# PaddlePaddle/Anakin

Hardware: AMD Instinct MI355X
Metric: ResNet50 INT8 images/sec + p50 latency @ batch 1/8, 1×MI355X (higher is better)
Workload: dtype int8

## Files before the change

### anakin_amd/build.py

```python
import os
import subprocess
import sys

HERE = os.path.dirname(os.path.abspath(__file__))
CSRC = os.path.join(HERE, "csrc")
LIB = os.path.join(HERE, "libsaber_mi355x.so")
SOURCES = ["conv_igemm.hip", "elementwise.hip", "fc_small.hip", "conv1x1_chain.hip", "conv_chain_coop.hip", "conv_stage_coop.hip", "stage_xcd.hip", "conv3x3_b3h.hip", "conv1x1_pw.hip", "conv1x1_pwk.hip", "conv_stem_f32.hip", "fc_f32_splitk.hip", "conv_dw3x3.hip", "conv_group3x3.hip", "conv_sep.hip"] + \
    ["api_%s.hip" % n for n in ("conv", "select", "autotune", "ops", "chain", "sep", "stage", "net", "net_optimize", "net_autotune", "capture", "gemm", "streams")] + \
    ["igemm_m%d_e%d.hip" % me for me in [(0, 0), (0, 1), (0, 2), (0, 3), (0, 4), (1, 0), (1, 1), (1, 2), (1, 3), (2, 3), (3, 3)]] + \
    ["igemm_dma_m%d_e%d.hip" % me for me in [(0, 0), (0, 1), (0, 2), (0, 3), (0, 4), (2, 3)]] + \
    ["halo_e%d.hip" % e for e in range(4)] + ["img_e%d.hip" % e for e in (0, 1, 3)] + ["stem_e%d.hip" % e for e in range(4)] + ["stem_pool.hip"]
FLAGS = ["--offload-arch=gfx950", "-O3", "-std=c++17", "-fPIC", "-ffp-contract=off", "-fno-fast-math",
         "-Wno-unused-result", "-mllvm", "-amdgpu-mfma-vgpr-form"]


def _stale(obj, deps):
    if not os.path.exists(obj):
        return True
    t = os.path.getmtime(obj)
    return any(os.path.getmtime(d) > t for d in deps)


def build(force=False, verbose=False):
    hipcc = os.environ.get("HIPCC", "/opt/rocm/bin/hipcc")
    objdir = os.path.join(HERE, "build")
    os.makedirs(objdir, exist_ok=True)
    import glob
    headers = sorted(glob.glob(os.path.join(CSRC, "*.h"))) + [os.path.join(HERE, "..", "include", "saber_hip.h")]
    objs = []
    procs = []
    for src in SOURCES:
        sp = os.path.join(CSRC, src)
        obj = os.path.join(objdir, src.replace(".hip", ".o"))
        objs.append(obj)
        deps = [h for h in headers if src.startswith("api_") or os.path.basename(h) != "api_internal.h"]
        if force or _stale(obj, [sp] + deps):
            cmd = [hipcc] + FLAGS + ["-c", sp, "-o", obj]
            if verbose:
                print(" ".join(cmd))
            procs.append((src, subprocess.Popen(cmd)))
    for src, p in procs:
        if p.wait() != 0:
            raise RuntimeError("hipcc failed on " + src)
    if force or procs or _stale(LIB, objs):
        cmd = [hipcc, "--offload-arch=gfx950", "-shared", "-o", LIB] + objs
        if verbose:
            print(" ".join(cmd))
        subprocess.check_call(cmd)
    return LIB


def build_cpp_tests(verbose=False):
    import glob
    root = os.path.dirname(HERE)
    build()
    subprocess.check_call(["make", "-s", "-C", os.path.join(root, "oracle"), "oracle"])
    hipcc = os.environ.get("HIPCC", "/opt/rocm/bin/hipcc")
    outs = []
    for src in sorted(glob.glob(os.path.join(root, "tests", "cpp", "*.cpp"))):
        out = src[:-4] + ".bin"
        deps = [src, os.path.join(root, "include", "saber_mi355x.hpp"), os.path.join(root, "include", "saber_mi355x_impl.h"), os.path.join(root, "include", "saber_hip.h"), LIB]
        if _stale(out, deps):
            cmd = [hipcc, "--offload-arch=gfx950", "-O2", "-std=c++17", "-I" + os.path.join(root, "include"), src, "-o", out,
                   "-L" + HERE, "-lsaber_mi355x", "-L" + os.path.join(root, "oracle"), "-lsaber_oracle",
                   "-Wl,-rpath,$ORIGIN/../../anakin_amd", "-Wl,-rpath,$ORIGIN/../../oracle", "-Wno-unused-result", "-mllvm", "-amdgpu-mfma-vgpr-form"]
            if verbose:
                print(" ".join(cmd))
            subprocess.check_call(cmd)
        outs.append(out)
    return outs


if __name__ == "__main__":
    print(build(force="--force" in sys.argv, verbose=True))
```

### anakin_amd/csrc/api_stage.hip

```cpp
#include "api_internal.h"

struct saber_hip_stage {
    std::vector<saber_hip_conv*> convs;
    std::vector<StagePhase> phases;
    DevBuf<uint8_t> d_phases, d_w, d_prm;
    DevBuf<unsigned long long> d_sync, d_trace;
    int n_barriers = 0, n_tensors = 0, n_img = 0, h = 0, w = 0;
    size_t lds_bytes = 0;
};

namespace {
constexpr int kSyncWords = 16 * 17 + 16;

bool stage_conv_ok(const saber_hip_conv* o) {
    const saber_hip_conv_desc& d = o->d;
    const bool k1 = d.kh == 1 && d.kw == 1 && d.pad_h == 0 && d.pad_w == 0;
    const bool k3 = d.kh == 3 && d.kw == 3 && d.pad_h == 1 && d.pad_w == 1;
    const bool res_ok = d.res_mode == SABER_HIP_RES_NONE ||
                        (d.res_mode == SABER_HIP_RES_ELTWISE && d.out_dtype == SABER_HIP_S8 &&
                         (!d.res_has_dtype || d.res_dtype == SABER_HIP_S8) && d.res_stride <= 1);
    return o->is_i8 && o->weights_set && o->algo == ALGO_IGEMM_I8 && o->epi == EPI_I8_CONV && (k1 || k3) && d.stride_h == 1 &&
           d.stride_w == 1 && d.dil_h == 1 && d.dil_w == 1 && d.group == 1 && !o->pair_k2 && !o->pool_fused && !o->pool2 &&
           !o->pre_quant && !o->pre_pad && o->c_eff == d.c && d.act_negative_slope == 0.f && d.in_layout == SABER_HIP_NHWC &&
           d.out_layout == SABER_HIP_NHWC && (d.out_dtype == SABER_HIP_S8 || d.out_dtype == SABER_HIP_U8) && res_ok &&
// ... 53 lines not shown
        if (i == 0) { st->n_img = d.n; st->h = d.h; st->w = d.w; }
        if (d.n != st->n_img || d.h != st->h || d.w != st->w || d.h * d.w > 64) return fail(SABER_HIP_INVALID_VALUE, "stage: all phases run on the same n x h x w, h * w <= 64");
        const int slots[4] = {ph[i].in, ph[i].out, elt ? ph[i].res : 0, ph[i].pool >= 0 ? ph[i].pool : 0};
        for (int s : slots)
            if (s < 0 || s >= STAGE_MAX_TENSORS) return fail(SABER_HIP_INVALID_VALUE, "stage: tensor slot out of range");
        if (ph[i].out == ph[i].in || (elt && ph[i].out == ph[i].res) || written[ph[i].out])
            return fail(SABER_HIP_INVALID_VALUE, "stage: every phase writes a slot of its own (no in-place, no rewrite)");
        const int taps = d.kh * d.kw, ksteps = d.c * taps / 64;
        const int nt = (d.k / 16 + 31) / 32;
        StagePhase p;
        std::memset(&p, 0, sizeof p);
        if (ksteps % 4 || !stage_xcd_type(nt, ksteps / 4, taps == 9, &p.type))
            return fail(SABER_HIP_INVALID_VALUE, "stage: no kernel variant for " + std::to_string(d.c) + " -> " + std::to_string(d.k) + (taps == 9 ? " 3x3" : " 1x1"));
        p.cin = d.c; p.cout = d.k;
        p.in_t = ph[i].in; p.out_t = ph[i].out; p.res_t = elt ? ph[i].res : -1;
        p.in_u8 = o->x_dtype == DT_U8;
        p.relu = d.act == SABER_HIP_ACT_RELU;
        p.out_u8 = d.out_dtype == SABER_HIP_U8;
        p.elt = elt;
        p.res_relu = d.res_act == SABER_HIP_ACT_RELU;
        p.coeff_conv = d.coeff_conv; p.scale_conv = o->out_scale; p.coeff_res = d.coeff_res; p.scale_res = d.scale_res;
        p.barrier = dirty[p.in_t] || (elt && dirty[p.res_t]);
        if (p.barrier) {
            std::fill(dirty.begin(), dirty.end(), 0);
            st->n_barriers += 1;
        }
        p.reload = (p.barrier || p.in_t != prev_in || i == 0) ? 1 : 0;
        prev_in = p.in_t;
        dirty[p.out_t] = written[p.out_t] = 1;
        p.pch = (unsigned)(d.c / 16 + 1);
        p.mg_pch = (unsigned)((0x100000000ull + p.pch - 1) / p.pch);
        const size_t a64 = ((size_t)(d.h * d.w + 1) * p.pch + 63) / 64 * 64;
        p.red_chunk = (int)a64;
        lds_chunks = std::max(lds_chunks, a64 + (size_t)4 * nt * 4 * 64 + (size_t)4 * nt * 4);
        p.pool_t = ph[i].pool;
        p.pool_idiv = 1.0f / (float)(d.h * d.w);
        p.w_chunk = (unsigned)(wbytes.size() / 16);
        pack_stage_weights(o, nt, ksteps / 4, wbytes);
        p.prm_chunk = (unsigned)(pbytes.size() / 16);
        const int kpad = 32 * nt * 16;
        const size_t base = pbytes.size();
        pbytes.resize(base + (size_t)kpad / 4 * 48, 0);
        for (int k = 0; k < d.k; ++k) {
            uint8_t* q = pbytes.data() + base + (size_t)(k / 4) * 48;
            ((float*)q)[k % 4] = o->scale_host.empty() ? 1.f : o->scale_host[k];
            ((float*)q)[4 + k % 4] = (o->has_bias && !o->bias_p_host.empty()) ? o->bias_p_host[k] : 0.f;
            ((int*)q)[8 + k % 4] = o->comp_host.empty() ? 0 : o->comp_host[k];
        }
        st->n_tensors = std::max(st->n_tensors, std::max(std::max(p.in_t, p.pool_t), std::max(p.out_t, p.res_t)) + 1);
        st->phases.push_back(p);
        st->convs.push_back(o);
    }
    st->lds_bytes = xcd_resident ? std::max<size_t>(lds_chunks * 16, 81 * 1024) : lds_chunks * 16;
    if (st->lds_bytes > 160 * 1024 - 64) return fail(SABER_HIP_UNIMPL, "stage: the image does not fit in LDS");
    std::vector<uint8_t> pt((const uint8_t*)st->phases.data(), (const uint8_t*)st->phases.data() + st->phases.size() * sizeof(StagePhase));
    hipError_t e = st->d_phases.upload(pt);
    if (e == hipSuccess) e = st->d_w.upload(wbytes);
    if (e == hipSuccess) e = st->d_prm.upload(pbytes);
    if (e == hipSuccess && xcd_resident) e = st->d_sync.alloc_zero(kSyncWords);
    if (e != hipSuccess) return hip_fail(e, "stage: device copies");
    if (!zero_page()) return fail(SABER_HIP_RUNTIME_ERROR, "stage: zero page");
    *out = st.release();
    return SABER_HIP_OK;
}
}

bool img_conv_ok(const saber_hip_conv* op) {
    if (!stage_conv_ok(op) || op->d.h * op->d.w > 64) return false;
    const int taps = op->d.kh * op->d.kw, ksteps = op->d.c * taps / 64;
    int type = 0;
    return ksteps % 4 == 0 && stage_xcd_type((op->d.k / 16 + 31) / 32, ksteps / 4, taps == 9, &type);
}
int img_conv_prepare(saber_hip_conv* op) {
    if (op->img_stage) return SABER_HIP_OK;
    if (!img_conv_ok(op)) return fail(SABER_HIP_INVALID_VALUE, "image-resident kernel: 1x1 / 3x3 stride-1 INT8 conv on <= 64 pixels per image with ResNet res5 channel shapes");
    const StageSpec sp = {op, 0, 1, op->d.res_mode == SABER_HIP_RES_ELTWISE ? 2 : -1, op->gpool ? 3 : -1};
    return stage_build(&sp, 1, false, &op->img_stage);
}
int img_conv_run(saber_hip_conv* op, const void* x, void* y, const void* res, void* y_pool, hipStream_t stream) {
    saber_hip_stage* st = op->img_stage;
    if (!st) return fail(SABER_HIP_INVALID_VALUE, "image-resident kernel selected without its buffers (set_tile / autotune build them)");
    const StagePhase& p = st->phases[0];
    if (!x || !y || (p.elt && !res) || (p.pool_t >= 0 && !y_pool)) return fail(SABER_HIP_INVALID_VALUE, "null tensor");
    StageKArgs k;
    std::memset(&k, 0, sizeof k);
    k.phases = (const StagePhase*)st->d_phases.p;
    k.weights = st->d_w.p; k.prm = st->d_prm.p; k.zero = zero_page();
    k.n_phases = 1;
    k.n_img = st->n_img; k.H = st->h; k.W = st->w;
    k.t[0] = const_cast<void*>(x); k.t[1] = y; k.t[2] = const_cast<void*>(res); k.t[3] = y_pool;
    HIP_TRY(launch_img_conv(k, st->lds_bytes, stream));
    return SABER_HIP_OK;
}
void img_conv_release(saber_hip_conv* op) {
    delete op->img_stage;
    op->img_stage = nullptr;
}

int saber_hip_stage_num_tensors(const saber_hip_stage_t* st) { return st ? st->n_tensors : 0; }

int saber_hip_stage_run(saber_hip_stage_t* st, void* const* tensors, int n_tensors, saber_hip_stream_t stream) {
    if (g_capture) return capture_unsupported("saber_hip_stage_run");
    if (!st || !tensors || n_tensors < st->n_tensors) return fail(SABER_HIP_INVALID_VALUE, "stage: tensor table too short");
    StageKArgs k;
    std::memset(&k, 0, sizeof k);
    k.phases = (const StagePhase*)st->d_phases.p;
    k.weights = st->d_w.p; k.prm = st->d_prm.p; k.zero = zero_page();
    k.sync = st->d_sync.p;
    k.n_phases = (int)st->phases.size(); k.n_barriers = st->n_barriers;
    k.n_img = st->n_img; k.H = st->h; k.W = st->w;
    k.trace = st->d_trace.p;
    for (int i = 0; i < st->n_tensors; ++i) k.t[i] = tensors[i];
    for (const StagePhase& p : st->phases)
        if (!k.t[p.in_t] || !k.t[p.out_t] || (p.elt && !k.t[p.res_t])) return fail(SABER_HIP_INVALID_VALUE, "stage: null tensor");
    HIP_TRY(launch_stage_xcd(k, st->lds_bytes, (hipStream_t)stream));
    return SABER_HIP_OK;
}

int saber_hip_stage_status(saber_hip_stage_t* st) {
    if (!st) return fail(SABER_HIP_INVALID_VALUE, "null argument");
    HIP_TRY(hipDeviceSynchronize());
    unsigned long long flag = 0;
    HIP_TRY(hipMemcpy(&flag, st->d_sync.p + 16 * 16, sizeof flag, hipMemcpyDeviceToHost));
    if (!flag) return SABER_HIP_OK;
    HIP_TRY(hipMemset(st->d_sync.p, 0, kSyncWords * sizeof(unsigned long long)));
    HIP_TRY(hipDeviceSynchronize());
    return fail(SABER_HIP_RUNTIME_ERROR, "stage: a workgroup gave up waiting for its XCD (the launch did not have the CUs to itself)");
}

int saber_hip_stage_trace(saber_hip_stage_t* st, unsigned long long* out, size_t cap) {
    if (!st) return fail(SABER_HIP_INVALID_VALUE, "null argument");
    const size_t n = (size_t)256 * st->phases.size() * 8;
    if (!out) {
        HIP_TRY(st->d_trace.alloc_zero(n));
        return (int)n;
    }
    if (!st->d_trace.p || cap < n) return fail(SABER_HIP_INVALID_VALUE, "stage trace: not armed / buffer too short");
    HIP_TRY(hipDeviceSynchronize());
    HIP_TRY(hipMemcpy(out, st->d_trace.p, n * sizeof(unsigned long long), hipMemcpyDeviceToHost));
    return (int)n;
}

void saber_hip_stage_destroy(saber_hip_stage_t* st) { delete st; }
```

### anakin_amd/csrc/fc_small.hip

```cpp
#include "conv_igemm_impl.h"

namespace saber_mi355x {

struct FcSoftmaxTail {
    float* prob;
    unsigned* ctr;
};
template <int KSW, bool SM, bool FENCED = false>
__device__ __forceinline__ void fc_i8_small_body(const ConvKArgs& a, const FcSoftmaxTail& t) {
    __shared__ v4i red[3][64];
    __shared__ unsigned last_flag;
    SABER_TL_DECL;
    SABER_TL(0);
    const int tid = threadIdx.x, lane = tid & 63;
    const int wave = __builtin_amdgcn_readfirstlane(tid >> 6);
    const int frow = lane & 15, fq = lane >> 4;
    const int n0 = blockIdx.x * 16;
    const int m = frow < a.M ? frow : a.M - 1;
    const char* wp = (const char*)a.w + (size_t)(n0 + frow) * a.Kg_pad + (size_t)wave * (KSW * 64) + fq * 16;
    const char* xp = (const char*)a.x + (size_t)m * a.C + (size_t)wave * (KSW * 64) + fq * 16;
    v4i wf[KSW], xf[KSW];
#pragma unroll
    for (int s = 0; s < KSW; ++s) wf[s] = *(const v4i*)(wp + s * 64);
#pragma unroll
    for (int s = 0; s < KSW; ++s) {
        const bool in = (wave * KSW + s) * 64 + fq * 16 < a.C;
        xf[s] = *(const v4i*)(in ? xp + s * 64 : (const char*)a.zero);
    }
    const int kb = n0 + fq * 4;
    ChanParams<4> cp;
    load_chan_params<4>(a, kb, cp);
    const int xmask = a.in_u8 ? (int)0x80808080u : 0;
    SABER_TL(1);
    v4i acc = {0, 0, 0, 0};
#pragma unroll
    for (int s = 0; s < KSW; ++s) {
        v4i b = xf[s];
        b.x ^= xmask; b.y ^= xmask; b.z ^= xmask; b.w ^= xmask;
        acc = mma_step(wf[s], b, acc);
    }
    SABER_TL(2);
    if (wave > 0) red[wave - 1][lane] = acc;
    __syncthreads();
    SABER_TL(3);
    if (wave == 0) {
        acc += red[0][lane];
        acc += red[1][lane];
        acc += red[2][lane];
        if (frow < a.M && kb < a.K) {
            float out[4];
#pragma unroll
            for (int r = 0; r < 4; ++r) {
                const int v = acc[r] + cp.comp[r];
                const float d = (float)v;
                if (a.epi == EPI_I8_FC_S8) out[r] = __fadd_rn(__fmul_rn(d, cp.scale[r]), cp.bias[r]);
                else out[r] = (cp.scale[r] == 1.f) ? d : __fmul_rn(cp.scale[r], d);
            }
            float* y = (float*)a.y + (size_t)frow * a.K + kb;
            if constexpr (SM) {
                for (int r = 0; r < 4; ++r)
                    if (kb + r < a.K) __hip_atomic_store(y + r, out[r], __ATOMIC_RELAXED, __HIP_MEMORY_SCOPE_AGENT);
            } else if (kb + 4 <= a.K && (a.K & 3) == 0) {
                *(float4*)y = make_float4(out[0], out[1], out[2], out[3]);
            } else {
                for (int r = 0; r < 4; ++r)
                    if (kb + r < a.K) y[r] = out[r];
            }
        }
    }
    SABER_TL(4);
    if constexpr (!SM) {
        SABER_TL_FLUSH();
        return;
    } else {
        if constexpr (FENCED) {
            asm volatile("s_waitcnt vmcnt(0)" ::: "memory");
            __syncthreads();
            if (tid == 0) {
                __builtin_amdgcn_fence(__ATOMIC_RELEASE, "agent");
                asm volatile("s_waitcnt vmcnt(0)" ::: "memory");
                last_flag = __hip_atomic_fetch_add(t.ctr, 1u, __ATOMIC_RELAXED, __HIP_MEMORY_SCOPE_AGENT) == gridDim.x - 1 ? 1u : 0u;
                if (last_flag) __builtin_amdgcn_fence(__ATOMIC_ACQUIRE, "agent");
            }
        } else if (wave == 0) {
            asm volatile("s_waitcnt vmcnt(0)" ::: "memory");
            if (lane == 0) last_flag = __hip_atomic_fetch_add(t.ctr, 1u, __ATOMIC_RELAXED, __HIP_MEMORY_SCOPE_AGENT) == gridDim.x - 1 ? 1u : 0u;
        }
        __syncthreads();
        if (!last_flag) {
            SABER_TL_FLUSH();
            return;
        }
        SABER_TL(5);
        if (tid == 0) __hip_atomic_store(t.ctr, 0u, __ATOMIC_RELAXED, __HIP_MEMORY_SCOPE_AGENT);
        constexpr int PER = 16;
        for (int row0 = wave; row0 < a.M; row0 += 8) {
            const int row1 = row0 + 4;
            const bool has1 = row1 < a.M;
            const float* y0 = (const float*)a.y + (size_t)row0 * a.K;
            const float* y1 = (const float*)a.y + (size_t)(has1 ? row1 : row0) * a.K;
            float v0[PER], v1[PER];
#pragma unroll
            for (int i = 0; i < PER; ++i) {
                const int c = lane + 64 * i;
                const int cc = c < a.K ? c : a.K - 1;
                v0[i] = __hip_atomic_load(y0 + cc, __ATOMIC_RELAXED, __HIP_MEMORY_SCOPE_SYSTEM);
                v1[i] = __hip_atomic_load(y1 + cc, __ATOMIC_RELAXED, __HIP_MEMORY_SCOPE_SYSTEM);
            }
            auto normalise = [&](float (&v)[PER], int row) {
                float mx = -3.4e38f;
#pragma unroll
                for (int i = 0; i < PER; ++i) mx = lane + 64 * i < a.K ? fmaxf(mx, v[i]) : mx;
#pragma unroll
                for (int o = 32; o > 0; o >>= 1) mx = fmaxf(mx, __shfl_xor(mx, o, 64));
                float sum = 0.f;
#pragma unroll
                for (int i = 0; i < PER; ++i) {
                    v[i] = lane + 64 * i < a.K ? expf(v[i] - mx) : 0.f;
                    sum += v[i];
                }
#pragma unroll
                for (int o = 32; o > 0; o >>= 1) sum += __shfl_xor(sum, o, 64);
                float* pr = t.prob + (size_t)row * a.K;
#pragma unroll
                for (int i = 0; i < PER; ++i)
                    if (lane + 64 * i < a.K) pr[lane + 64 * i] = v[i] / sum;
            };
            normalise(v0, row0);
            if (has1) normalise(v1, row1);
        }
        SABER_TL(6);
        SABER_TL_FLUSH();
    }
}
template <int KSW>
__global__ __launch_bounds__(256) void fc_i8_small_kernel(const ConvKArgs a) {
    fc_i8_small_body<KSW, false>(a, FcSoftmaxTail{nullptr, nullptr});
}
template <int KSW, bool FENCED>
__global__ __launch_bounds__(256) void fc_i8_small_softmax_kernel(const ConvKArgs a, const FcSoftmaxTail t) {
    fc_i8_small_body<KSW, true, FENCED>(a, t);
}

struct FcStreamArgs {
    const float* w;
    const float* x;
    float* y;
    const float* bias;
    const void* zero;
    int m, n, c, w_pitch;
    int w_rows;
    int relu;
    float neg_slope, alpha, beta;
};

template <int NS, int NW, bool PACKED>
__global__ __launch_bounds__(NW * 64) void fc_f32_stream_kernel(const FcStreamArgs a) {
    __shared__ v4f redf[NW - 1][64];
    const int tid = threadIdx.x, lane = tid & 63;
    const int wave = __builtin_amdgcn_readfirstlane(tid >> 6);
    const int frow = lane & 15, fq = lane >> 4;
    const int n0 = blockIdx.x * 16;
    const int m = frow < a.m ? frow : a.m - 1;
    const int wr = n0 + frow < a.w_rows ? n0 + frow : a.w_rows - 1;
    const int ksw = (a.c + NW * 16 - 1) / (NW * 16);
    const int k0 = wave * ksw * 16 + fq * 4;
    const float* const wrow = PACKED ? a.w + ((size_t)blockIdx.x * a.w_pitch * 64 + lane) * 4 : a.w + (size_t)wr * a.w_pitch;
    const float* const xrow = a.x + (size_t)m * a.c;
    const float* const zero = (const float*)a.zero;
    v4f acc[4];
#pragma unroll
    for (int i = 0; i < 4; ++i) acc[i] = v4f{0.f, 0.f, 0.f, 0.f};
    v4i wf[2][NS], xf[2][NS];
    auto request = [&](int b, int s0) {
#pragma unroll
        for (int s = 0; s < NS; ++s) {
            const int k = k0 + (s0 + s) * 16;
            const bool in = s0 + s < ksw && k < a.c;
            const float* wp = PACKED ? wrow + (size_t)(s0 + s < ksw ? wave * ksw + s0 + s : wave * ksw) * 256 : (in ? wrow + k : wrow);
            const float* xp = in ? xrow + k : zero;
            wf[b][s] = __builtin_nontemporal_load((const v4i*)wp);
            xf[b][s] = *(const v4i*)xp;
        }
    };
    auto multiply = [&](int b) {
#pragma unroll
        for (int s = 0; s < NS; ++s) {
            const v4f wv = __builtin_bit_cast(v4f, wf[b][s]);
            const v4f xv = __builtin_bit_cast(v4f, xf[b][s]);
            acc[0] = __builtin_amdgcn_mfma_f32_16x16x4f32(wv.x, xv.x, acc[0], 0, 0, 0);
            acc[1] = __builtin_amdgcn_mfma_f32_16x16x4f32(wv.y, xv.y, acc[1], 0, 0, 0);
            acc[2] = __builtin_amdgcn_mfma_f32_16x16x4f32(wv.z, xv.z, acc[2], 0, 0, 0);
            acc[3] = __builtin_amdgcn_mfma_f32_16x16x4f32(wv.w, xv.w, acc[3], 0, 0, 0);
        }
    };
    const int nch = (ksw + NS - 1) / NS;
    const int rot = (int)((blockIdx.x * 7u + wave * 3u) % (unsigned)nch);
    auto chunk_s0 = [&](int ci) { return ci < nch ? ((ci + rot) % nch) * NS : ksw; };
    request(0, chunk_s0(0));
    __builtin_amdgcn_sched_barrier(0);
    for (int ci = 0; ci < nch; ci += 2) {
        request(1, chunk_s0(ci + 1));
        __builtin_amdgcn_sched_barrier(0);
        multiply(0);
        __builtin_amdgcn_sched_barrier(0);
        request(0, chunk_s0(ci + 2));
        __builtin_amdgcn_sched_barrier(0);
        multiply(1);
        __builtin_amdgcn_sched_barrier(0);
    }
    v4f sum = (acc[0] + acc[1]) + (acc[2] + acc[3]);
    if (wave > 0) redf[wave - 1][lane] = sum;
    __syncthreads();
    if (wave > 0) return;
#pragma unroll
    for (int w = 0; w < NW - 1; ++w) sum += redf[w][lane];
    const int kb = n0 + fq * 4;
    if (frow >= a.m || kb >= a.n) return;
    float* y = a.y + (size_t)frow * a.n + kb;
    float out[4];
#pragma unroll
    for (int r = 0; r < 4; ++r) {
        float d = a.alpha == 1.f ? sum[r] : __fmul_rn(a.alpha, sum[r]);
// ... 87 lines not shown
#pragma unroll
    for (int r = 0; r < 4; ++r) {
        float d = a.alpha == 1.f ? sum[r] : __fmul_rn(a.alpha, sum[r]);
        if (a.bias && kb + r < a.n) d = __fadd_rn(d, a.bias[kb + r]);
        if (a.relu) d = d > 0.f ? d : (a.neg_slope == 0.f ? 0.f : __fmul_rn(d, a.neg_slope));
        if (a.beta != 0.f && kb + r < a.n) d = __fadd_rn(d, __fmul_rn(a.beta, y[r]));
        out[r] = d;
    }
    if (kb + 4 <= a.n && (a.n & 3) == 0) {
        *(float4*)y = make_float4(out[0], out[1], out[2], out[3]);
    } else {
        for (int r = 0; r < 4; ++r)
            if (kb + r < a.n) y[r] = out[r];
    }
}

bool fc_f32_small_ok(int m, int c, int kg_pad) { return m >= 1 && m <= 16 && c % 4 == 0 && c <= 65536 && kg_pad >= (c + 63) / 64 * 64; }
static hipError_t launch_fc_f32_stream(const FcStreamArgs& f, bool packed, hipStream_t s) {
    const dim3 grid((f.n + 15) / 16);
    const bool deep = (f.c + 63) / 64 >= 48;
    if (packed) {
        if (deep) hipLaunchKernelGGL((fc_f32_stream_kernel<12, 4, true>), grid, dim3(256), 0, s, f);
        else hipLaunchKernelGGL((fc_f32_stream_kernel<4, 4, true>), grid, dim3(256), 0, s, f);
    } else {
        if (deep) hipLaunchKernelGGL((fc_f32_stream_kernel<12, 4, false>), grid, dim3(256), 0, s, f);
        else hipLaunchKernelGGL((fc_f32_stream_kernel<4, 4, false>), grid, dim3(256), 0, s, f);
    }
    return hipGetLastError();
}
hipError_t launch_fc_f32_small(const ConvKArgs& a, bool packed, hipStream_t s) {
    if (!fc_f32_small_ok(a.M, a.C, a.Kg_pad)) return hipErrorInvalidValue;
    FcStreamArgs f;
    f.w = (const float*)a.w; f.x = (const float*)a.x; f.y = (float*)a.y; f.bias = a.bias; f.zero = a.zero;
    f.m = a.M; f.n = a.K; f.c = a.C;
    f.w_pitch = packed ? fc_f32_packed_steps(a.C) : a.Kg_pad;
    f.w_rows = (a.K + 15) / 16 * 16;
    f.relu = a.relu; f.neg_slope = a.neg_slope; f.alpha = 1.f; f.beta = 0.f;
    if (!packed && a.C >= 2048) {
        const dim3 grid((f.n + 15) / 16), block(256);
        if (f.m <= 8) hipLaunchKernelGGL((gemm_f32_rows_lds_kernel<8>), grid, block, 0, s, f);
        else hipLaunchKernelGGL((gemm_f32_rows_lds_kernel<16>), grid, block, 0, s, f);
        return hipGetLastError();
    }
    return launch_fc_f32_stream(f, packed, s);
}
int fc_f32_packed_steps(int c) { return 4 * ((c + 63) / 64); }
bool gemm_f32_rows_ok(int m, int k) { return m >= 1 && m <= 16 && k % 4 == 0 && k <= (1 << 24); }
hipError_t launch_gemm_f32_rows(int m, int n, int k, float alpha, const float* A, const float* B, float beta, float* C, const void* zero,
                                hipStream_t s) {
    if (!gemm_f32_rows_ok(m, k)) return hipErrorInvalidValue;
    FcStreamArgs f;
    f.w = B; f.x = A; f.y = C; f.bias = nullptr; f.zero = zero;
    f.m = m; f.n = n; f.c = k; f.w_pitch = k; f.w_rows = n;
    f.relu = 0; f.neg_slope = 0.f; f.alpha = alpha; f.beta = beta;
    static const bool gather = [] { const char* e = std::getenv("SABER_HIP_GEMM_ROWS_GATHER"); return e && e[0] == '1'; }();
    if (k >= 2048 && !gather) {
        const dim3 grid((n + 15) / 16), block(256);
        if (m <= 8) hipLaunchKernelGGL((gemm_f32_rows_lds_kernel<8>), grid, block, 0, s, f);
        else hipLaunchKernelGGL((gemm_f32_rows_lds_kernel<16>), grid, block, 0, s, f);
        return hipGetLastError();
    }
    return launch_fc_f32_stream(f, false, s);
}

bool fc_i8_small_ok(int m, int c, int kg_pad) { return m >= 1 && m <= 16 && c % 16 == 0 && c <= 4 * 16 * 64 && kg_pad >= ((c + 255) / 256) * 256; }

hipError_t launch_fc_i8_small(const ConvKArgs& a, hipStream_t s) {
    if (!fc_i8_small_ok(a.M, a.C, a.Kg_pad)) return hipErrorInvalidValue;
    const int ksw = (a.C + 255) / 256;
    dim3 grid((a.K + 15) / 16), block(256);
#define SABER_FC_CASE(n) case n: hipLaunchKernelGGL((fc_i8_small_kernel<n>), grid, block, 0, s, a); break;
    switch (ksw) {
        SABER_FC_CASE(1) SABER_FC_CASE(2) SABER_FC_CASE(3) SABER_FC_CASE(4) SABER_FC_CASE(5) SABER_FC_CASE(6)
        SABER_FC_CASE(7) SABER_FC_CASE(8) SABER_FC_CASE(9) SABER_FC_CASE(10) SABER_FC_CASE(11) SABER_FC_CASE(12)
        SABER_FC_CASE(13) SABER_FC_CASE(14) SABER_FC_CASE(15) SABER_FC_CASE(16)
    default: return hipErrorInvalidValue;
    }
#undef SABER_FC_CASE
    return hipGetLastError();
}
bool fc_i8_small_softmax_ok(int m, int c, int kg_pad, int k) { return fc_i8_small_ok(m, c, kg_pad) && k >= 1 && k <= 1024; }
hipError_t launch_fc_i8_small_softmax(const ConvKArgs& a, float* prob, unsigned* ctr, hipStream_t s) {
    if (!fc_i8_small_softmax_ok(a.M, a.C, a.Kg_pad, a.K) || !prob || !ctr) return hipErrorInvalidValue;
    const int ksw = (a.C + 255) / 256;
    dim3 grid((a.K + 15) / 16), block(256);
    const FcSoftmaxTail t{prob, ctr};
    static const bool fenced = [] { const char* e = std::getenv("SABER_HIP_FC_SOFTMAX_FENCED"); return e && e[0] == '1'; }();
#define SABER_FC_CASE(n) case n: if (fenced) hipLaunchKernelGGL((fc_i8_small_softmax_kernel<n, true>), grid, block, 0, s, a, t); \
                                 else hipLaunchKernelGGL((fc_i8_small_softmax_kernel<n, false>), grid, block, 0, s, a, t); break;
    switch (ksw) {
        SABER_FC_CASE(2) SABER_FC_CASE(4) SABER_FC_CASE(8) SABER_FC_CASE(16)
    default: return hipErrorInvalidValue;
    }
#undef SABER_FC_CASE
    return hipGetLastError();
}

}
```

### anakin_amd/csrc/kernels.h

```cpp
#pragma once
#include <hip/hip_runtime.h>
#include <stddef.h>
#include <stdint.h>

#ifdef SABER_TIMELINE
extern __device__ unsigned long long* saber_tl_buf;
#define SABER_TL_DECL unsigned long long tl_[16] = {0, 0, 0, 0, 0, 0, 0, 0, 0, 0, 0, 0, 0, 0, 0, 0}
#define SABER_TL(i) tl_[i] = wall_clock64()
#define SABER_TL_FLUSH()                                                                   \
    do {                                                                                   \
        if (threadIdx.x == 0 && saber_tl_buf)                                              \
            for (int i_ = 0; i_ < 16; ++i_) saber_tl_buf[(size_t)blockIdx.x * 16 + i_] = tl_[i_]; \
    } while (0)
#else
#define SABER_TL_DECL do { } while (0)
#define SABER_TL(i) do { } while (0)
#define SABER_TL_FLUSH() do { } while (0)
#endif

namespace saber_mi355x {

enum { DT_F32 = 0, DT_S8 = 1, DT_U8 = 2 };

enum {
// ... 88 lines not shown
    int tiles_x, tiles_per_img;
    unsigned mg_tiles_x, mg_tpi;
    int in0_u8, relu0;
    int s0, H0, W0;
    int res_sub, res_H, res_W;
    void* y2b;
    int k2_split, relu2b, out_u8_2b;
};
struct CoopKArgs {
    ChainKArgs c;
    unsigned long long* coop_ctr;
    void* coop_xch;
    unsigned* coop_xcc;
    unsigned* coop_err;
    int n_tiles;
};
bool conv1x1_chain_ok(int c1, int k1, int k2);
hipError_t launch_conv1x1_chain(const ChainKArgs& a, int c1, int k1, int k2, int rows, int waves, int split, int with3x3, hipStream_t s);
hipError_t launch_conv_chain_coop(const CoopKArgs& a, hipStream_t s);

struct StageBlk {
    const void* wstream;
    const void* prm0;
    const void* prm1;
    const void* prm2;
    float coeff_conv, scale_conv, coeff_res, scale_res;
    int in0_u8, relu0, in_u8, relu1, res_relu, relu2, out_u8_2, pad_;
};
template <int MAXB>
struct Stage4KArgs {
    const void* x;
    const void* res;
    const void* zero;
    const StageBlk* blk;
    unsigned long long* grp_ctr;
    unsigned long long* img_ctr;
    void* xch;
    unsigned* xcc;
    unsigned* err;
    int nblk, N, H, W;
    int tiles_x, tiles_per_img;
    unsigned mg_tiles_x, mg_tpi, mg_wpi;
    int per_image;
    void* y1[MAXB];
    void* y2[MAXB];
    void* head_y;
};
constexpr int STAGE4_SHORT = 8, STAGE4_LONG = 24;
hipError_t launch_conv_stage4(const Stage4KArgs<STAGE4_SHORT>& a, bool tail, bool head, hipStream_t s);
hipError_t launch_conv_stage4(const Stage4KArgs<STAGE4_LONG>& a, bool tail, bool head, hipStream_t s);
hipError_t launch_conv_stage1_c128(const Stage4KArgs<STAGE4_SHORT>& a, hipStream_t s);
hipError_t launch_conv_stage1_c128(const Stage4KArgs<STAGE4_LONG>& a, hipStream_t s);

struct StagePhase {
    int type;
    int cin, cout;
    int in_t, out_t, res_t;
    int in_u8, relu, out_u8;
    int elt, res_relu;
    float coeff_conv, scale_conv, coeff_res, scale_res;
    unsigned w_chunk, prm_chunk;
    int barrier;
    int reload;
    unsigned pch, mg_pch;
    int red_chunk;
    int pool_t;
    float pool_idiv;
};
static_assert(sizeof(StagePhase) == 96, "StagePhase layout");
struct StageKArgs {
    const StagePhase* phases;
    const void* weights;
    const void* prm;
    const void* zero;
    unsigned long long* sync;
    int n_phases, n_barriers;
    int n_img, H, W;
    unsigned long long* trace;
    void* t[STAGE_MAX_TENSORS];
};
bool stage_xcd_type(int tiles_per_cu, int ksteps_per_wave, int is3x3, int* type);
hipError_t launch_stage_xcd(const StageKArgs& a, size_t lds_bytes, hipStream_t s);
hipError_t launch_img_conv(const StageKArgs& a, size_t lds_bytes, hipStream_t s);

__device__ __forceinline__ void pin_hot_args(const ConvKArgs& a) {
    asm volatile("" ::"s"(a.x), "s"(a.w), "s"(a.zero), "s"(a.npx), "s"(a.nky), "s"(a.mg_npx), "s"(a.Kg_pad), "s"(a.M), "s"(a.OH),
                 "s"(a.OW), "s"(a.inv_ohw), "s"(a.inv_ow), "s"(a.H), "s"(a.W), "s"(a.C), "s"(a.stride_h), "s"(a.stride_w),
                 "s"(a.pad_h), "s"(a.pad_w), "s"(a.dil_h), "s"(a.dil_w), "s"(a.kh), "s"(a.kw), "s"(a.steps), "s"(a.in_u8));
}

enum { TILE_32x32 = 0, TILE_64x32 = 1, TILE_64x64 = 2, TILE_128x64 = 3, TILE_64x128 = 4, TILE_128x128 = 5,
       TILE_COUNT = 6,
       TILE_W8_64x64 = 6, TILE_W8_128x64 = 7, TILE_W8_128x128 = 8, TILE_W8_256x128 = 9, TILE_COUNT_B3 = 10 };
void tile_dims(int tile, int* bm_k, int* bn_pix);

hipError_t launch_conv_igemm(int mode, int tile, int ks, const ConvKArgs& a, hipStream_t s);
hipError_t launch_conv_igemm_dma(int mode, int tile, int ks, int wg, const ConvKArgs& a, hipStream_t s);
hipError_t launch_conv3x3_halo(int th, const ConvKArgs& a, hipStream_t s);
hipError_t launch_conv3x3_img(const ConvKArgs& a, int nw, int ib, int rb, hipStream_t s);
bool conv3x3_img_feasible(int C, int OW, int OH, int N, int nw, int ib, int rb);
bool conv3x3_b3h_variant(int variant, int* bmk, int* th, int* tm, int* threads);
bool conv1x1_pw_ok(int c, int k);
hipError_t launch_conv1x1_pw(const ConvKArgs& a, hipStream_t s);
bool conv1x1_pwk_variant(int v, int* tm, int* p, int* d, int* minb);
bool conv1x1_pwk_ok(int m, int c, int k);
hipError_t launch_conv1x1_pwk(int variant, const ConvKArgs& a, hipStream_t s);
hipError_t launch_conv3x3_b3h(int variant, const ConvKArgs& a, hipStream_t s);
hipError_t launch_fc_i8_small(const ConvKArgs& a, hipStream_t s);
bool fc_i8_small_ok(int m, int c, int kg_pad);
hipError_t launch_fc_f32_small(const ConvKArgs& a, bool packed, hipStream_t s);
int fc_f32_packed_steps(int c);
bool fc_f32_small_ok(int m, int c, int kg_pad);
bool fc_i8_small_softmax_ok(int m, int c, int kg_pad, int k);
hipError_t launch_fc_i8_small_softmax(const ConvKArgs& a, float* prob, unsigned* ctr, hipStream_t s);
bool fc_f32_splitk_ok(int m, int c, int kg_pad, int k, bool softmax);
size_t fc_f32_splitk_part_floats(int c, int k);
size_t fc_f32_splitk_counters(int k);
hipError_t launch_fc_f32_splitk(const ConvKArgs& a, float* part, unsigned* ctr, float* prob, hipStream_t s);
bool gemm_f32_rows_ok(int m, int k);
hipError_t launch_gemm_f32_rows(int m, int n, int k, float alpha, const float* A, const float* B, float beta, float* C, const void* zero,
                                hipStream_t s);
hipError_t launch_conv_stem(int f32_in, const ConvKArgs& a, hipStream_t s);
hipError_t launch_conv_stem_pool(int f32_in, const ConvKArgs& a, hipStream_t s);
hipError_t launch_conv_stem_pool_pair(int f32_in, const StemPairKArgs& a, hipStream_t s);
hipError_t launch_conv_direct(int is_f32, const ConvKArgs& a, int group, hipStream_t s);
constexpr int DW3X3_FORMS = 2;
const char* conv_dw3x3_form_name(int form, bool f32);
bool conv_dw3x3_ok(bool f32, int n, int c, int k, int group, int kh, int kw, int stride_h, int stride_w, int pad_h, int pad_w, int dil_h,
                   int dil_w, int oh, int ow);
hipError_t launch_conv_dw3x3(int form, bool f32, const ConvKArgs& a, hipStream_t s);
constexpr int G3X3_FORMS = 1;
const char* conv_group3x3_form_name(int form);
int conv_group3x3_steps(int cg);
bool conv_group3x3_ok(int n, int c, int k, int group, int kh, int kw, int stride_h, int stride_w, int pad_h, int pad_w, int dil_h, int dil_w,
                      int oh, int ow);
hipError_t launch_conv_group3x3(int form, const ConvKArgs& a, int group, hipStream_t s);

struct SepKArgs {
    const void* x;
    const void* wdw;
    const float* dw_bias;
    const float* dw_scale;
    const void* wpw;
    const void* prm;
    void* y_dw;
    void* y_pw;
    int N, H, W, C, OH, OW, K;
    int stride, pad;
    int tiles_x, tiles_per_img;
    int kgroups;
    int nslices;
    int dw_relu, mid_u8;
    int pw_relu, out_u8;
};
constexpr int SEP_MAX_CODE = 15;
bool conv_sep_form(int code, int* rows, int* kper, int* waves);
bool conv_sep_form_ok(int code, int c, int k);
size_t conv_sep_lds_bytes(int rows, int c);
void sep_pw_pack(const int8_t* w_kc, int k, int c, std::vector<uint8_t>& out);
hipError_t conv_sep_prepare();
hipError_t launch_conv_sep(int code, bool in_u8, const SepKArgs& a, hipStream_t s);

hipError_t launch_l2_flush(const void* buf, size_t bytes, unsigned* sink, hipStream_t s);

hipError_t launch_quantize_nchw_to_nhwc(int n, int c, int h, int w, int c_pad, int out_dtype, float scale,
                                        const float* x, void* y, hipStream_t s);
// ... 36 lines not shown
```

### anakin_amd/csrc/stage_xcd.hip

```cpp
#include "epilogue_pack.h"

namespace saber_mi355x {

namespace {

typedef const __attribute__((address_space(4))) StagePhase* PhasePtr;

__device__ __forceinline__ unsigned stage_xcc_id() {
    unsigned v;
    asm volatile("s_getreg_b32 %0, hwreg(HW_REG_XCC_ID)" : "=s"(v));
    return v & 7u;
}
__device__ __forceinline__ unsigned long long stage_sload(const unsigned long long* p) {
    unsigned long long v;
    asm volatile("s_dcache_inv\n\ts_load_dwordx2 %0, %1, 0x0\n\ts_waitcnt lgkmcnt(0)" : "=&s"(v) : "s"(p) : "memory");
    return v;
}
__device__ __forceinline__ void stage_dma16(const void* src, void* dst_wave_base) {
    __builtin_amdgcn_global_load_lds((const __attribute__((address_space(1))) void*)src,
                                     (__attribute__((address_space(3))) void*)dst_wave_base, 16, 0, 0);
}
__device__ __forceinline__ void stage_dma16_l2(const void* src, void* dst_wave_base) {
    __builtin_amdgcn_global_load_lds((const __attribute__((address_space(1))) void*)src,
                                     (__attribute__((address_space(3))) void*)dst_wave_base, 16, 0, 16);
// ... 185 lines not shown
                unsigned w = 0;
#pragma unroll
                for (int t = 0; t < 4; ++t) {
                    const float f = rintf(__fmul_rn((float)tot[t], php->pool_idiv));
                    const int q = u8o ? (int)fminf(fmaxf(f, 0.f), 255.f) : (int)fminf(fmaxf(f, -128.f), 127.f);
                    w |= (unsigned)(q & 0xff) << (8 * t);
                }
                if (ch < cout) *(unsigned*)((char*)a.t[pool_t] + (size_t)img * cout + ch) = w;
            }
        }
    }
    STAGE_TR(7);
#undef STAGE_TR
    return true;
}

}

__global__ __launch_bounds__(256) void stage_xcd_kernel(const StageKArgs a) {
    extern __shared__ v4i stage_lds[];
    __shared__ unsigned s_x, s_idx, s_abort;
    __shared__ unsigned long long s_gen;
    const int tid = threadIdx.x;
    if (tid == 0) {
        const unsigned x = stage_xcc_id();
        const unsigned long long me = __hip_atomic_fetch_add(a.sync + 16 * x, 1ull, __ATOMIC_RELAXED, __HIP_MEMORY_SCOPE_AGENT);
        s_x = x;
        s_idx = (unsigned)(me & 31ull);
        s_gen = me >> 5;
        s_abort = 0u;
    }
    __syncthreads();
    StageCtx cx;
    cx.xcd = (int)s_x;
    cx.cu = (int)s_idx;
    cx.gen = s_gen;
    cx.ctr = a.sync + 16 * (8 + cx.xcd);
    cx.abort_w = a.sync + 16 * 16;
    cx.bar = 0;
    cx.hw = a.H * a.W;
    cx.img0 = cx.xcd;
    cx.img_step = 8;
    if (cx.xcd >= a.n_img) {
        if (tid == 0 && a.n_barriers) __hip_atomic_fetch_add(cx.ctr, (unsigned long long)a.n_barriers, __ATOMIC_RELAXED, __HIP_MEMORY_SCOPE_AGENT);
        return;
    }
    const int frow = tid & 15;
#pragma unroll
    for (int m = 0; m < 4; ++m) {
        const int p = m * 16 + frow;
        cx.py[m] = p < cx.hw ? p / a.W : -1;
        cx.px[m] = p < cx.hw ? p - (p / a.W) * a.W : 0;
    }
    PhasePtr tab = (PhasePtr)a.phases;
    for (int p = 0; p < a.n_phases; ++p) {
        PhasePtr php = tab + p;
        cx.tr = a.trace ? a.trace + ((size_t)blockIdx.x * a.n_phases + p) * 8 : nullptr;
        bool ok = false;
        switch (php->type) {
        case 0: ok = stage_phase<4, 4, false>(a, php, cx, stage_lds, &s_abort); break;
        case 1: ok = stage_phase<1, 4, false>(a, php, cx, stage_lds, &s_abort); break;
        case 2: ok = stage_phase<1, 18, true>(a, php, cx, stage_lds, &s_abort); break;
        case 3: ok = stage_phase<4, 2, false>(a, php, cx, stage_lds, &s_abort); break;
        case 4: ok = stage_phase<1, 8, false>(a, php, cx, stage_lds, &s_abort); break;
        default: break;
        }
        if (!ok) return;
    }
}

__global__ __launch_bounds__(256) void img_conv_kernel(const StageKArgs a) {
    extern __shared__ v4i stage_lds[];
    __shared__ unsigned s_abort;
    StageCtx cx;
    cx.xcd = 0;
    cx.cu = (int)(blockIdx.x & 31u);
    cx.gen = 0;
    cx.ctr = nullptr;
    cx.abort_w = nullptr;
    cx.bar = 0;
    cx.hw = a.H * a.W;
    cx.img0 = (int)(blockIdx.x >> 5);
    cx.img_step = 1 << 30;
    cx.tr = nullptr;
    const int frow = threadIdx.x & 15;
#pragma unroll
    for (int m = 0; m < 4; ++m) {
        const int p = m * 16 + frow;
        cx.py[m] = p < cx.hw ? p / a.W : -1;
        cx.px[m] = p < cx.hw ? p - (p / a.W) * a.W : 0;
    }
    PhasePtr php = (PhasePtr)a.phases;
    switch (php->type) {
    case 0: (void)stage_phase<4, 4, false>(a, php, cx, stage_lds, &s_abort); break;
    case 1: (void)stage_phase<1, 4, false>(a, php, cx, stage_lds, &s_abort); break;
    case 2: (void)stage_phase<1, 18, true>(a, php, cx, stage_lds, &s_abort); break;
    case 3: (void)stage_phase<4, 2, false>(a, php, cx, stage_lds, &s_abort); break;
    case 4: (void)stage_phase<1, 8, false>(a, php, cx, stage_lds, &s_abort); break;
    default: break;
    }
}

bool stage_xcd_type(int tiles_per_cu, int ksteps_per_wave, int is3x3, int* type) {
    static const int tab[5][3] = {{4, 4, 0}, {1, 4, 0}, {1, 18, 1}, {4, 2, 0}, {1, 8, 0}};
    for (int i = 0; i < 5; ++i)
        if (tab[i][0] == tiles_per_cu && tab[i][1] == ksteps_per_wave && tab[i][2] == is3x3) {
            *type = i;
            return true;
        }
    return false;
}

hipError_t launch_stage_xcd(const StageKArgs& a, size_t lds_bytes, hipStream_t s) {
    if (lds_bytes > 160 * 1024 - 64 || lds_bytes <= 80 * 1024) return hipErrorInvalidValue;
    static bool done[64] = {false};
    int dev = 0;
    hipError_t e = hipGetDevice(&dev);
    if (e != hipSuccess || dev < 0 || dev >= 64) return e != hipSuccess ? e : hipErrorInvalidDevice;
    if (!done[dev]) {
        e = hipFuncSetAttribute((const void*)stage_xcd_kernel, hipFuncAttributeMaxDynamicSharedMemorySize, 160 * 1024 - 64);
        if (e != hipSuccess) return e;
        done[dev] = true;
    }
    hipLaunchKernelGGL(stage_xcd_kernel, dim3(256), dim3(256), lds_bytes, s, a);
    return hipGetLastError();
}

hipError_t launch_img_conv(const StageKArgs& a, size_t lds_bytes, hipStream_t s) {
    if (lds_bytes > 160 * 1024 - 64 || a.n_img <= 0 || a.n_img > (1 << 20)) return hipErrorInvalidValue;
    static bool done[64] = {false};
    int dev = 0;
    hipError_t e = hipGetDevice(&dev);
    if (e != hipSuccess || dev < 0 || dev >= 64) return e != hipSuccess ? e : hipErrorInvalidDevice;
    if (!done[dev]) {
        e = hipFuncSetAttribute((const void*)img_conv_kernel, hipFuncAttributeMaxDynamicSharedMemorySize, 160 * 1024 - 64);
        if (e != hipSuccess) return e;
        done[dev] = true;
    }
    hipLaunchKernelGGL(img_conv_kernel, dim3(a.n_img * 32), dim3(256), lds_bytes, s, a);
    return hipGetLastError();
}

}
```

Baseline: 38460.

## Add dedicated 1x1 conv+global-pool kernel and widen FC softmax to 512 threads

Adds a specialized kernel for the final ResNet 1x1 conv (512->2048, <=64 pixels) fused with residual add and global average pooling. It loads the whole image into LDS and keeps weights in registers, and replaces the generic image-resident stage kernel for that layer. It also changes the FC+softmax kernel to 8 waves with half the K-split per wave, uses 128-bit buffer stores for logits, and simplifies the softmax row loop. A timeline trace pointer is enabled in the img kernel under a debug macro.

```diff
diff --git a/anakin_amd/build.py b/anakin_amd/build.py
--- a/anakin_amd/build.py
+++ b/anakin_amd/build.py
@@ -5,7 +5,7 @@
 HERE = os.path.dirname(os.path.abspath(__file__))
 CSRC = os.path.join(HERE, "csrc")
 LIB = os.path.join(HERE, "libsaber_mi355x.so")
-SOURCES = ["conv_igemm.hip", "elementwise.hip", "fc_small.hip", "conv1x1_chain.hip", "conv_chain_coop.hip", "conv_stage_coop.hip", "stage_xcd.hip", "conv3x3_b3h.hip", "conv1x1_pw.hip", "conv1x1_pwk.hip", "conv_stem_f32.hip", "fc_f32_splitk.hip", "conv_dw3x3.hip", "conv_group3x3.hip", "conv_sep.hip"] + \
+SOURCES = ["conv_igemm.hip", "elementwise.hip", "fc_small.hip", "conv1x1_chain.hip", "conv_chain_coop.hip", "conv_stage_coop.hip", "stage_xcd.hip", "conv1x1_gpool.hip", "conv3x3_b3h.hip", "conv1x1_pw.hip", "conv1x1_pwk.hip", "conv_stem_f32.hip", "fc_f32_splitk.hip", "conv_dw3x3.hip", "conv_group3x3.hip", "conv_sep.hip"] + \
     ["api_%s.hip" % n for n in ("conv", "select", "autotune", "ops", "chain", "sep", "stage", "net", "net_optimize", "net_autotune", "capture", "gemm", "streams")] + \
     ["igemm_m%d_e%d.hip" % me for me in [(0, 0), (0, 1), (0, 2), (0, 3), (0, 4), (1, 0), (1, 1), (1, 2), (1, 3), (2, 3), (3, 3)]] + \
     ["igemm_dma_m%d_e%d.hip" % me for me in [(0, 0), (0, 1), (0, 2), (0, 3), (0, 4), (2, 3)]] + \
diff --git a/anakin_amd/csrc/api_stage.hip b/anakin_amd/csrc/api_stage.hip
--- a/anakin_amd/csrc/api_stage.hip
+++ b/anakin_amd/csrc/api_stage.hip
@@ -159,6 +159,18 @@
     if (!st) return fail(SABER_HIP_INVALID_VALUE, "image-resident kernel selected without its buffers (set_tile / autotune build them)");
     const StagePhase& p = st->phases[0];
     if (!x || !y || (p.elt && !res) || (p.pool_t >= 0 && !y_pool)) return fail(SABER_HIP_INVALID_VALUE, "null tensor");
+    if (p.pool_t >= 0 && op->d.kh == 1 && conv1x1_gpool_ok(p.cin, p.cout, st->h * st->w)) {
+        GpoolKArgs g;
+        std::memset(&g, 0, sizeof g);
+        g.x = x; g.y = y; g.res = p.elt ? res : nullptr; g.y_pool = y_pool;
+        g.w = st->d_w.p + (size_t)p.w_chunk * 16; g.prm = st->d_prm.p + (size_t)p.prm_chunk * 16; g.zero = zero_page();
+        g.n_img = st->n_img; g.hw = st->h * st->w; g.cout = p.cout;
+        g.in_u8 = p.in_u8; g.relu = p.relu; g.out_u8 = p.out_u8; g.elt = p.elt; g.res_relu = p.res_relu;
+        g.coeff_conv = p.coeff_conv; g.scale_conv = p.scale_conv; g.coeff_res = p.coeff_res; g.scale_res = p.scale_res;
+        g.pool_idiv = p.pool_idiv;
+        HIP_TRY(launch_conv1x1_gpool(g, stream));
+        return SABER_HIP_OK;
+    }
     StageKArgs k;
     std::memset(&k, 0, sizeof k);
     k.phases = (const StagePhase*)st->d_phases.p;
diff --git a/anakin_amd/csrc/conv1x1_gpool.hip b/anakin_amd/csrc/conv1x1_gpool.hip
--- /dev/null
+++ b/anakin_amd/csrc/conv1x1_gpool.hip
@@ -0,0 +1,131 @@
+#include "epilogue_pack.h"
+
+namespace saber_mi355x {
+
+namespace {
+constexpr int kCin = 512, kPch = kCin / 16 + 1;
+constexpr int kImgChunks = ((64 + 1) * kPch + 63) / 64 * 64;
+}
+
+__global__ __launch_bounds__(256) void conv1x1_gpool_kernel(const GpoolKArgs a) {
+    __shared__ v4i img_lds[kImgChunks];
+    SABER_TL_DECL;
+    SABER_TL(0);
+    asm volatile("" ::"s"(a.x), "s"(a.y), "s"(a.res), "s"(a.y_pool), "s"(a.w), "s"(a.prm), "s"(a.zero), "s"(a.hw), "s"(a.cout),
+                 "s"(a.in_u8), "s"(a.relu), "s"(a.out_u8), "s"(a.elt), "s"(a.res_relu), "s"(a.coeff_conv), "s"(a.scale_conv),
+                 "s"(a.coeff_res), "s"(a.scale_res), "s"(a.pool_idiv));
+    const int tid = threadIdx.x, lane = tid & 63;
+    const int wave = __builtin_amdgcn_readfirstlane(tid >> 6);
+    const int frow = lane & 15, fq = lane >> 4;
+    const int cu = (int)(blockIdx.x & 31u), img = (int)(blockIdx.x >> 5);
+    const int HW = a.hw, cout = a.cout;
+    {
+        const char* xg = (const char*)a.x + (size_t)img * HW * kCin;
+        const int nA = (int)(((unsigned)(HW + 1) * kPch + 63u) / 64u);
+        for (int i = wave; i < nA; i += 4) {
+            const unsigned L = (unsigned)(i * 64 + lane);
+            const unsigned hp = L / (unsigned)kPch, cc = L - hp * kPch;
+            const bool in = hp < (unsigned)HW && cc < (unsigned)(kCin / 16);
+            const char* src = in ? xg + (size_t)hp * kCin + cc * 16 : (const char*)a.zero;
+            lds_dma16(src, img_lds + i * 64);
+        }
+    }
+    v4i wreg[8];
+    {
+        const v4i* wp = (const v4i*)a.w + lane;
+#pragma unroll
+        for (int ks = 0; ks < 8; ++ks) wreg[ks] = wp[(size_t)((cu * 4 + ks / 2) * 8 + (ks % 2) * 4 + wave) * 64];
+    }
+    const int ch = cu * 64 + wave * 16 + fq * 4;
+    const bool ch_ok = ch < cout;
+    v4i prm[3];
+    {
+        const v4i* pp = (const v4i*)a.prm + (ch / 4) * 3;
+#pragma unroll
+        for (int r = 0; r < 3; ++r) prm[r] = pp[r];
+    }
+    const bool elt = a.elt != 0;
+    unsigned rs[4] = {0u, 0u, 0u, 0u};
+    if (elt) {
+#pragma unroll
+        for (int m = 0; m < 4; ++m) {
+            const int p = m * 16 + frow;
+            const char* rp = (p < HW && ch_ok) ? (const char*)a.res + ((size_t)img * HW + p) * cout + ch : (const char*)a.zero;
+            rs[m] = *(const unsigned*)rp;
+        }
+    }
+    SABER_TL(1);
+    asm volatile("s_waitcnt vmcnt(0)" ::: "memory");
+    __syncthreads();
+    SABER_TL(2);
+    const int xmask = a.in_u8 ? (int)0x80808080u : 0;
+    v4i acc[4];
+#pragma unroll
+    for (int m = 0; m < 4; ++m) acc[m] = v4i{0, 0, 0, 0};
+#pragma unroll
+    for (int ks = 0; ks < 8; ++ks) {
+        v4i bf[4];
+#pragma unroll
+        for (int m = 0; m < 4; ++m) {
+            const int p = m * 16 + frow;
+            const int q = p < HW ? p : HW;
+            v4i b = img_lds[q * kPch + ks * 4 + fq];
+            b.x ^= xmask; b.y ^= xmask; b.z ^= xmask; b.w ^= xmask;
+            bf[m] = b;
+        }
+#pragma unroll
+        for (int m = 0; m < 4; ++m) acc[m] = mma_step(wreg[ks], bf[m], acc[m]);
+    }
+    SABER_TL(3);
+    const float lo = a.relu ? 0.f : -3.0e38f;
+    const float off = a.out_u8 ? 0.f : 128.f;
+    const unsigned xo = a.out_u8 ? 0u : 0x80808080u;
+    const float lo_s8 = a.relu ? 0.f : -128.f;
+    const float res_lo = a.res_relu ? 0.f : -3.0e38f;
+    struct { float coeff_conv, scale_conv, coeff_res, scale_res; } ec = {a.coeff_conv, a.scale_conv, a.coeff_res, a.scale_res};
+    const bool u8o = a.out_u8 && !elt;
+    char* yout = (char*)a.y + (size_t)img * HW * cout + ch;
+    int ps[4] = {0, 0, 0, 0};
+#pragma unroll
+    for (int m = 0; m < 4; ++m) {
+        const int p = m * 16 + frow;
+        unsigned o;
+        if (elt) o = chain_elt_pack(acc[m], prm[2], __builtin_bit_cast(v4f, prm[1]), __builtin_bit_cast(v4f, prm[0]), rs[m], lo_s8, res_lo, ec);
+        else o = chain_out_pack(acc[m], prm[2], __builtin_bit_cast(v4f, prm[1]), __builtin_bit_cast(v4f, prm[0]), lo, off, xo);
+        if (p < HW && ch_ok) *(unsigned*)(yout + (size_t)p * cout) = o;
+#pragma unroll
+        for (int t = 0; t < 4; ++t) {
+            const int b = (int)((o >> (8 * t)) & 0xffu);
+            const int v = u8o ? b : (int)(int8_t)b;
+            ps[t] += p < HW ? v : 0;
+        }
+    }
+    SABER_TL(4);
+#pragma unroll
+    for (int t = 0; t < 4; ++t)
+#pragma unroll
+        for (int s = 1; s < 16; s <<= 1) ps[t] += __shfl_xor(ps[t], s, 64);
+    if (frow == 0 && ch_ok) {
+        unsigned w = 0;
+#pragma unroll
+        for (int t = 0; t < 4; ++t) {
+            const float f = rintf(__fmul_rn((float)ps[t], a.pool_idiv));
+            const int q = u8o ? (int)fminf(fmaxf(f, 0.f), 255.f) : (int)fminf(fmaxf(f, -128.f), 127.f);
+            w |= (unsigned)(q & 0xff) << (8 * t);
+        }
+        *(unsigned*)((char*)a.y_pool + (size_t)img * cout + ch) = w;
+    }
+    SABER_TL(5);
+    SABER_TL_FLUSH();
+}
+
+bool conv1x1_gpool_ok(int cin, int cout, int hw) { return cin == kCin && cout % 16 == 0 && cout > 1536 && cout <= 2048 && hw >= 1 && hw <= 64; }
+
+hipError_t launch_conv1x1_gpool(const GpoolKArgs& a, hipStream_t s) {
+    if (!conv1x1_gpool_ok(kCin, a.cout, a.hw) || a.n_img <= 0 || a.n_img > (1 << 20)) return hipErrorInvalidValue;
+    if (!a.x || !a.y || !a.y_pool || !a.w || !a.prm || !a.zero || (a.elt && !a.res)) return hipErrorInvalidValue;
+    hipLaunchKernelGGL(conv1x1_gpool_kernel, dim3(a.n_img * 32), dim3(256), 0, s, a);
+    return hipGetLastError();
+}
+
+}
diff --git a/anakin_amd/csrc/fc_small.hip b/anakin_amd/csrc/fc_small.hip
--- a/anakin_amd/csrc/fc_small.hip
+++ b/anakin_amd/csrc/fc_small.hip
@@ -1,6 +1,8 @@
 #include "conv_igemm_impl.h"
 
 namespace saber_mi355x {
+
+typedef unsigned v4u __attribute__((ext_vector_type(4)));
 
 struct FcSoftmaxTail {
     float* prob;
@@ -8,7 +10,8 @@
 };
 template <int KSW, bool SM, bool FENCED = false>
 __device__ __forceinline__ void fc_i8_small_body(const ConvKArgs& a, const FcSoftmaxTail& t) {
-    __shared__ v4i red[3][64];
+    constexpr int NW = SM ? 8 : 4;
+    __shared__ v4i red[NW - 1][64];
     __shared__ unsigned last_flag;
     SABER_TL_DECL;
     SABER_TL(0);
@@ -44,9 +47,8 @@
     __syncthreads();
     SABER_TL(3);
     if (wave == 0) {
-        acc += red[0][lane];
-        acc += red[1][lane];
-        acc += red[2][lane];
+#pragma unroll
+        for (int w = 0; w < NW - 1; ++w) acc += red[w][lane];
         if (frow < a.M && kb < a.K) {
             float out[4];
 #pragma unroll
@@ -58,8 +60,14 @@
             }
             float* y = (float*)a.y + (size_t)frow * a.K + kb;
             if constexpr (SM) {
-                for (int r = 0; r < 4; ++r)
-                    if (kb + r < a.K) __hip_atomic_store(y + r, out[r], __ATOMIC_RELAXED, __HIP_MEMORY_SCOPE_AGENT);
+                if (kb + 4 <= a.K && (a.K & 3) == 0) {
+                    const __amdgpu_buffer_rsrc_t yr = __builtin_amdgcn_make_buffer_rsrc(a.y, 0, 0xffffffff, 0x00020000);
+                    const v4f o4 = {out[0], out[1], out[2], out[3]};
+                    __builtin_amdgcn_raw_buffer_store_b128(__builtin_bit_cast(v4u, o4), yr, (int)(((unsigned)frow * (unsigned)a.K + (unsigned)kb) * 4u), 0, 16);
+                } else {
+                    for (int r = 0; r < 4; ++r)
+                        if (kb + r < a.K) __hip_atomic_store(y + r, out[r], __ATOMIC_RELAXED, __HIP_MEMORY_SCOPE_AGENT);
+                }
             } else if (kb + 4 <= a.K && (a.K & 3) == 0) {
                 *(float4*)y = make_float4(out[0], out[1], out[2], out[3]);
             } else {
@@ -94,40 +102,32 @@
         SABER_TL(5);
         if (tid == 0) __hip_atomic_store(t.ctr, 0u, __ATOMIC_RELAXED, __HIP_MEMORY_SCOPE_AGENT);
         constexpr int PER = 16;
-        for (int row0 = wave; row0 < a.M; row0 += 8) {
-            const int row1 = row0 + 4;
-            const bool has1 = row1 < a.M;
-            const float* y0 = (const float*)a.y + (size_t)row0 * a.K;
-            const float* y1 = (const float*)a.y + (size_t)(has1 ? row1 : row0) * a.K;
-            float v0[PER], v1[PER];
+        for (int row = wave; row < a.M; row += NW) {
+            const float* y0 = (const float*)a.y + (size_t)row * a.K;
+            float v[PER];
 #pragma unroll
             for (int i = 0; i < PER; ++i) {
                 const int c = lane + 64 * i;
                 const int cc = c < a.K ? c : a.K - 1;
-                v0[i] = __hip_atomic_load(y0 + cc, __ATOMIC_RELAXED, __HIP_MEMORY_SCOPE_SYSTEM);
-                v1[i] = __hip_atomic_load(y1 + cc, __ATOMIC_RELAXED, __HIP_MEMORY_SCOPE_SYSTEM);
+                v[i] = __hip_atomic_load(y0 + cc, __ATOMIC_RELAXED, __HIP_MEMORY_SCOPE_SYSTEM);
             }
-            auto normalise = [&](float (&v)[PER], int row) {
-                float mx = -3.4e38f;
-#pragma unroll
-                for (int i = 0; i < PER; ++i) mx = lane + 64 * i < a.K ? fmaxf(mx, v[i]) : mx;
-#pragma unroll
-                for (int o = 32; o > 0; o >>= 1) mx = fmaxf(mx, __shfl_xor(mx, o, 64));
-                float sum = 0.f;
-#pragma unroll
-                for (int i = 0; i < PER; ++i) {
-                    v[i] = lane + 64 * i < a.K ? expf(v[i] - mx) : 0.f;
-                    sum += v[i];
-                }
-#pragma unroll
-                for (int o = 32; o > 0; o >>= 1) sum += __shfl_xor(sum, o, 64);
-                float* pr = t.prob + (size_t)row * a.K;
-#pragma unroll
-                for (int i = 0; i < PER; ++i)
-                    if (lane + 64 * i < a.K) pr[lane + 64 * i] = v[i] / sum;
-            };
-            normalise(v0, row0);
-            if (has1) normalise(v1, row1);
+            float mx = -3.4e38f;
+#pragma unroll
+            for (int i = 0; i < PER; ++i) mx = lane + 64 * i < a.K ? fmaxf(mx, v[i]) : mx;
+#pragma unroll
+            for (int o = 32; o > 0; o >>= 1) mx = fmaxf(mx, __shfl_xor(mx, o, 64));
+            float sum = 0.f;
+#pragma unroll
+            for (int i = 0; i < PER; ++i) {
+                v[i] = lane + 64 * i < a.K ? expf(v[i] - mx) : 0.f;
+                sum += v[i];
+            }
+#pragma unroll
+            for (int o = 32; o > 0; o >>= 1) sum += __shfl_xor(sum, o, 64);
+            float* pr = t.prob + (size_t)row * a.K;
+#pragma unroll
+            for (int i = 0; i < PER; ++i)
+                if (lane + 64 * i < a.K) pr[lane + 64 * i] = v[i] / sum;
         }
         SABER_TL(6);
         SABER_TL_FLUSH();
@@ -138,7 +138,7 @@
     fc_i8_small_body<KSW, false>(a, FcSoftmaxTail{nullptr, nullptr});
 }
 template <int KSW, bool FENCED>
-__global__ __launch_bounds__(256) void fc_i8_small_softmax_kernel(const ConvKArgs a, const FcSoftmaxTail t) {
+__global__ __launch_bounds__(512) void fc_i8_small_softmax_kernel(const ConvKArgs a, const FcSoftmaxTail t) {
     fc_i8_small_body<KSW, true, FENCED>(a, t);
 }
 
@@ -392,14 +392,15 @@
 bool fc_i8_small_softmax_ok(int m, int c, int kg_pad, int k) { return fc_i8_small_ok(m, c, kg_pad) && k >= 1 && k <= 1024; }
 hipError_t launch_fc_i8_small_softmax(const ConvKArgs& a, float* prob, unsigned* ctr, hipStream_t s) {
     if (!fc_i8_small_softmax_ok(a.M, a.C, a.Kg_pad, a.K) || !prob || !ctr) return hipErrorInvalidValue;
-    const int ksw = (a.C + 255) / 256;
-    dim3 grid((a.K + 15) / 16), block(256);
+    const int ksw = (a.C + 255) / 256 / 2;
+    if (((a.C + 255) / 256) & 1) return hipErrorInvalidValue;
+    dim3 grid((a.K + 15) / 16), block(512);
     const FcSoftmaxTail t{prob, ctr};
     static const bool fenced = [] { const char* e = std::getenv("SABER_HIP_FC_SOFTMAX_FENCED"); return e && e[0] == '1'; }();
 #define SABER_FC_CASE(n) case n: if (fenced) hipLaunchKernelGGL((fc_i8_small_softmax_kernel<n, true>), grid, block, 0, s, a, t); \
                                  else hipLaunchKernelGGL((fc_i8_small_softmax_kernel<n, false>), grid, block, 0, s, a, t); break;
     switch (ksw) {
-        SABER_FC_CASE(2) SABER_FC_CASE(4) SABER_FC_CASE(8) SABER_FC_CASE(16)
+        SABER_FC_CASE(1) SABER_FC_CASE(2) SABER_FC_CASE(4) SABER_FC_CASE(8)
     default: return hipErrorInvalidValue;
     }
 #undef SABER_FC_CASE
diff --git a/anakin_amd/csrc/kernels.h b/anakin_amd/csrc/kernels.h
--- a/anakin_amd/csrc/kernels.h
+++ b/anakin_amd/csrc/kernels.h
@@ -194,6 +194,21 @@
 bool stage_xcd_type(int tiles_per_cu, int ksteps_per_wave, int is3x3, int* type);
 hipError_t launch_stage_xcd(const StageKArgs& a, size_t lds_bytes, hipStream_t s);
 hipError_t launch_img_conv(const StageKArgs& a, size_t lds_bytes, hipStream_t s);
+struct GpoolKArgs {
+    const void* x;
+    void* y;
+    const void* res;
+    void* y_pool;
+    const void* w;
+    const void* prm;
+    const void* zero;
+    int n_img, hw, cout;
+    int in_u8, relu, out_u8, elt, res_relu;
+    float coeff_conv, scale_conv, coeff_res, scale_res;
+    float pool_idiv;
+};
+bool conv1x1_gpool_ok(int cin, int cout, int hw);
+hipError_t launch_conv1x1_gpool(const GpoolKArgs& a, hipStream_t s);
 
 __device__ __forceinline__ void pin_hot_args(const ConvKArgs& a) {
     asm volatile("" ::"s"(a.x), "s"(a.w), "s"(a.zero), "s"(a.npx), "s"(a.nky), "s"(a.mg_npx), "s"(a.Kg_pad), "s"(a.M), "s"(a.OH),
diff --git a/anakin_amd/csrc/stage_xcd.hip b/anakin_amd/csrc/stage_xcd.hip
--- a/anakin_amd/csrc/stage_xcd.hip
+++ b/anakin_amd/csrc/stage_xcd.hip
@@ -291,7 +291,11 @@
     cx.hw = a.H * a.W;
     cx.img0 = (int)(blockIdx.x >> 5);
     cx.img_step = 1 << 30;
+#ifdef SABER_TIMELINE
+    cx.tr = saber_tl_buf ? saber_tl_buf + (size_t)blockIdx.x * 16 : nullptr;
+#else
     cx.tr = nullptr;
+#endif
     const int frow = threadIdx.x & 15;
 #pragma unroll
     for (int m = 0; m < 4; ++m) {
```

Result: faster. 39260, median of 6 (+2.1%).
